# play-with-HOI-generation/HOIG

Hardware: AMD Instinct MI355X
Metric: HOGAN train images/sec at 256x256 (higher is better)
Workload: dtype f16x3 fwd (both operands split hi+lo on fp16, 3 MFMAs per product) / bf16x2 bwd (dy split hi+lo, weights and x single bf16, 2 MFMAs per product), f32 accumulate; 1 GPU; 256x256 HO3Dv3-shaped synthetic, batch 8 per GPU, G+D full step (generator_spade_attn, VGG19 surrogate weights); global_batch=8, parallelism=dp1

## Files before the change

hoig_amd/csrc/conv_route.h:

```cpp
#pragma once

#define HOIG_CONV_ROUTES(W, D, F, FD)                                                                                              \
          \
    W(wgrad_thin_in_ws) W(wgrad_thin_in_direct) W(wgrad_thin_out_ws) W(wgrad_thin_out_direct)                                      \
    W(wgrad_small)                                                                                                                 \
                                                                                        \
    W(wgrad_flat5) W(wgrad_tile5)                                                                                                  \
                                                                 \
    W(wgrad_halo_th4) W(wgrad_halo_cm2) W(wgrad_halo_cm1) W(wgrad_halo_s2_cm2) W(wgrad_halo_s2_cm1) W(wgrad_halo_5x5)              \
    W(wgrad_halo_tout)        \
                                                                                                  \
    W(wgrad_dma) W(wgrad_dma_pair)                                                                                                 \
    W(wgrad_bf16_64) W(wgrad_bf16_128)                                                                                             \
                                                                                 \
    W(wgrad_f32_32x64) W(wgrad_f32_32x128) W(wgrad_f32_64x128) W(wgrad_f32_128x64) W(wgrad_f32_128x128)                            \
                                                                                 \
    FD(igemm_f32_128x32) FD(igemm_f32_128x64) FD(igemm_f32_64x64) FD(igemm_f32_128x128) FD(igemm_f32_64x128)                       \
                       \
    FD(halo1_64) FD(halo1_128w) FD(halo1_128) FD(same5_64) FD(same5_128w) FD(same5_128)                                            \
                                                                                                             \
    FD(halo3_64) FD(halo3_128w) FD(halo3_128)                                                                                      \
         \
    FD(halo3_m16_64) FD(halo3_m16_128)                                                                                             \
    D(halo3_m16_64_split) D(halo3_m16_128_split) D(halo3_m16_64_split_pair) D(halo3_m16_128_split_pair)                            \
    F(halo3_m16_64_pair) F(halo3_m16_128_pair) F(halo3_m16_64_normin) F(halo3_m16_128_normin)                                      \
                                                   \
    FD(flat_m16_k3) FD(flat_m16_k5) FD(halo5_m16) FD(halo5_m16_ksplit)                                                             \
     \
    FD(s2g_64) FD(s2g_128) FD(s2s_64) FD(s2s_128)                                                                                  \
    FD(s2g_m16_64) FD(s2g_m16_128) FD(s2s_m16_64) FD(s2s_m16_128)                                                                  \
    FD(s2g_m16p4_64) FD(s2g_m16p4_128) FD(s2s_m16p4_64) FD(s2s_m16p4_128) FD(s2g_m16p8_128) FD(s2s_m16p8_128)                      \
                   \
    FD(igemm_m16_128x128) FD(igemm_m16_128x128w) FD(igemm_m16_64x128) FD(igemm_m16_128x64) FD(igemm_m16_64x64)                     \
    FD(igemm_bf16_128x128) FD(igemm_bf16_128x128w) FD(igemm_bf16_64x128) FD(igemm_bf16_128x64) FD(igemm_bf16_64x64)                \
                                                                                \
    D(k128) D(thin) D(thin_out) D(small)                                                                                           \
    F(head7) F(small) F(small_ci) F(dot) F(thin) F(thin_out)                                                                       \
// ... 27 lines not shown
```

hoig_amd/csrc/conv_thin.hip:

```cpp
#include "common.h"
#include <map>
#include <mutex>

namespace {

typedef _Float16 f16x8 __attribute__((ext_vector_type(8)));
typedef short s16x4 __attribute__((ext_vector_type(4)));

constexpr int TH = 4, TW = 32, NTHR = 256;

struct ThinArgs {
    const float *T;
    const float *D;
    const float *bias;
    float *Out;
    float *Ws;
    int Bn, H, W, F, CD, KS, pad;
    int flip;
    int sj, st, sf;
    int act;
    float slope;
    int accumulate;
    float wscale;
    int K, KP, N, NP;
    int tiles_x, tiles_y, ntiles, strip;
    int HR, CW;
    double *stats;
};

template <bool FP16>
__device__ __forceinline__ void split16(float x, unsigned short &hi, unsigned short &lo) {
    if (FP16) {
        const _Float16 h = (_Float16)x;
        const _Float16 l = (_Float16)(x - (float)h);
        hi = __builtin_bit_cast(unsigned short, h);
        lo = __builtin_bit_cast(unsigned short, l);
    } else {
        const __bf16 h = (__bf16)x;
        hi = __builtin_bit_cast(unsigned short, h);
        const __bf16 l = (__bf16)(x - hoig_bf2f(hi));
        lo = __builtin_bit_cast(unsigned short, l);
    }
}

template <bool FP16>
__device__ __forceinline__ f32x16 mfma16(const bf16x8 a, const bf16x8 b, const f32x16 c) {
    if (FP16) return __builtin_amdgcn_mfma_f32_32x32x16_f16(__builtin_bit_cast(f16x8, a), __builtin_bit_cast(f16x8, b), c, 0, 0, 0);
    return __builtin_amdgcn_mfma_f32_32x32x16_bf16(a, b, c, 0, 0, 0);
}

constexpr int HMAX = 12;
struct HaloRegs {
    float v[HMAX];
};
struct HaloMap {
    int lds[HMAX];
    int rc[HMAX];
    int rounds;
};
__device__ __forceinline__ void halo_map(const ThinArgs &p, HaloMap &m) {
    const int wr = TW + p.KS - 1;
    const int row_elems = wr * p.F;
    const int total = p.HR * row_elems;
    m.rounds = (total + NTHR - 1) / NTHR;
#pragma unroll
    for (int it = 0; it < HMAX; ++it) {
        const int i = threadIdx.x + it * NTHR;
        m.lds[it] = -1;
        m.rc[it] = 0;
        if (i < total) {
            const int hy = i / row_elems, e = i - hy * row_elems;
            const int hx = e / p.F, f = e - hx * p.F;
            m.lds[it] = (f * p.HR + hy) * p.CW + hx;
            m.rc[it] = hy | (hx << 8) | (f << 16);
        }
    }
}
__device__ __forceinline__ void halo_load(const ThinArgs &p, const HaloMap &m, int b, int y0, int x0, HaloRegs &h) {
    const float *img = p.T + (size_t)b * p.H * p.W * p.F;
#pragma unroll
    for (int it = 0; it < HMAX; ++it) {
        h.v[it] = 0.f;
        if (it < m.rounds && m.lds[it] >= 0) {
            const int gy = y0 - p.pad + (m.rc[it] & 255), gx = x0 - p.pad + ((m.rc[it] >> 8) & 255);
            if (gy >= 0 && gy < p.H && gx >= 0 && gx < p.W) h.v[it] = img[((size_t)gy * p.W + gx) * p.F + (m.rc[it] >> 16)];
        }
    }
}
template <bool FP16, int NT>
__device__ __forceinline__ void halo_store(const ThinArgs &p, const HaloMap &m, const HaloRegs &h, unsigned short *Tl) {
    const int plane = p.F * p.HR * p.CW;
#pragma unroll
    for (int it = 0; it < HMAX; ++it)
        if (it < m.rounds && m.lds[it] >= 0) {
            unsigned short hi, lo;
            split16<FP16>(h.v[it], hi, lo);
            Tl[m.lds[it]] = hi;
            if (NT == 2) Tl[plane + m.lds[it]] = lo;
        }
}

__device__ __forceinline__ void tile_coords(const ThinArgs &p, int t, int &b, int &y0, int &x0) {
    const int tx = t % p.tiles_x;
    t /= p.tiles_x;
    const int ty = t % p.tiles_y;
    b = t / p.tiles_y;
    y0 = ty * TH;
    x0 = tx * TW;
}

template <bool FP16, int NT, int NW>
__global__ __launch_bounds__(NTHR) void thin_gemm_kernel(const ThinArgs p) {
    extern __shared__ __attribute__((aligned(16))) unsigned char smem[];
    const int wstride = p.KP + 8;
    unsigned short *Wl = reinterpret_cast<unsigned short *>(smem);
    unsigned short *toff = Wl + NW * 64 * wstride;
    unsigned short *Tl = toff + p.KP;
    const int tid = threadIdx.x, lane = tid & 63, wave = tid >> 6;
    const int l31 = lane & 31, lh = lane >> 5;
    const int cbase = blockIdx.y * 64;
    const int KK = p.KS * p.KS;
    const int tplane = p.F * p.HR * p.CW;

    for (int i0 = tid; i0 < 64 * p.KP; i0 += 4 * NTHR) {
        float v[4];
        int dst[4];
#pragma unroll
        for (int u = 0; u < 4; ++u) {
            const int i = i0 + u * NTHR;
            v[u] = 0.f;
            dst[u] = -1;
            if (i < 64 * p.KP) {
                const int n = i / p.KP, k = i - n * p.KP;
                dst[u] = n * wstride + k;
                if (k < p.K) {
                    const int tap = k / p.F, f = k - tap * p.F;
                    const int tw = p.flip ? KK - 1 - tap : tap;
                    v[u] = p.D[(size_t)(cbase + n) * p.sj + (size_t)tw * p.st + (size_t)f * p.sf];
                }
            }
        }
#pragma unroll
        for (int u = 0; u < 4; ++u)
            if (dst[u] >= 0) {
                unsigned short hi, lo;
                split16<FP16>(v[u] * p.wscale, hi, lo);
                Wl[dst[u]] = hi;
                if (NW == 2) Wl[64 * wstride + dst[u]] = lo;
            }
    }
    for (int k = tid; k < p.KP; k += NTHR) {
        const int kc = k < p.K ? k : p.K - 1;
        const int tap = kc / p.F, f = kc - tap * p.F;
        const int r = tap / p.KS, s = tap - r * p.KS;
        toff[k] = (unsigned short)((f * p.HR + r) * p.CW + s);
    }

    const float nslope = p.act == HOIG_ACT_NONE ? 1.f : (p.act == HOIG_ACT_RELU ? 0.f : p.slope);
    const bool special = p.act == HOIG_ACT_TANH || p.act == HOIG_ACT_SIGMOID;
    const float inv = 1.f / p.wscale;
    float bias_r[2];
#pragma unroll
    for (int j = 0; j < 2; ++j) bias_r[j] = p.bias ? p.bias[cbase + j * 32 + l31] : 0.f;
    const int ksteps = p.KP >> 4;
    const int pix = wave * p.CW + l31;

    const int t_end = min(p.ntiles, (int)(blockIdx.x + 1) * p.strip);
    HaloRegs hreg;
    HaloMap hmap;
    halo_map(p, hmap);
    {
        int b, y0, x0;
        tile_coords(p, blockIdx.x * p.strip, b, y0, x0);
        halo_load(p, hmap, b, y0, x0, hreg);
    }
    float st1[2] = {0.f, 0.f}, st2[2] = {0.f, 0.f};
    int sb = -1;
    auto flush_stats = [&]() {
        if (sb >= 0) {
#pragma unroll
            for (int j = 0; j < 2; ++j) {
                const float s1 = st1[j] + __shfl_xor(st1[j], 32), s2 = st2[j] + __shfl_xor(st2[j], 32);
                if (lh == 0) {
                    hoig_stats_add(p.stats, sb, p.CD, 0, cbase + j * 32 + l31, s1);
                    hoig_stats_add(p.stats, sb, p.CD, 1, cbase + j * 32 + l31, s2);
                }
                st1[j] = st2[j] = 0.f;
            }
        }
    };
    for (int t = blockIdx.x * p.strip; t < t_end; ++t) {
        int b, y0, x0;
        tile_coords(p, t, b, y0, x0);
        if (p.stats && b != sb) {
            flush_stats();
            sb = b;
        }
        __syncthreads();
        halo_store<FP16, NT>(p, hmap, hreg, Tl);
        __syncthreads();
        if (t + 1 < t_end) {
            int b2, y2, x2;
            tile_coords(p, t + 1, b2, y2, x2);
            halo_load(p, hmap, b2, y2, x2, hreg);
        }
        f32x16 acc[2];
#pragma unroll
        for (int j = 0; j < 2; ++j)
#pragma unroll
            for (int r = 0; r < 16; ++r) acc[j][r] = 0.f;
#pragma unroll 1
        for (int kk = 0; kk < ksteps; ++kk) {
            const int k0 = kk * 16 + lh * 8;
            const bf16x8 offs = *reinterpret_cast<const bf16x8 *>(toff + k0);
            bf16x8 a0, a1;
#pragma unroll
            for (int e = 0; e < 8; ++e) {
                const int o = (int)(unsigned short)offs[e] + pix;
                a0[e] = (short)Tl[o];
                if (NT == 2) a1[e] = (short)Tl[tplane + o];
            }
#pragma unroll
            for (int j = 0; j < 2; ++j) {
                const unsigned short *wr = Wl + (j * 32 + l31) * wstride + k0;
                const bf16x8 w0 = *reinterpret_cast<const bf16x8 *>(wr);
                if (NT == 2) acc[j] = mfma16<FP16>(a1, w0, acc[j]);
                if (NW == 2) acc[j] = mfma16<FP16>(a0, *reinterpret_cast<const bf16x8 *>(wr + 64 * wstride), acc[j]);
                acc[j] = mfma16<FP16>(a0, w0, acc[j]);
            }
        }
        const int oy = y0 + wave;
#pragma unroll
        for (int r = 0; r < 16; ++r) {
            const int ox = x0 + (r & 3) + 8 * (r >> 2) + 4 * lh;
            float *dst = p.Out + (((size_t)b * p.H + oy) * p.W + ox) * p.CD + cbase + l31;
#pragma unroll
            for (int j = 0; j < 2; ++j) {
                float v = acc[j][r] * inv + bias_r[j];
                v = fast_act(v, nslope, special, p.act, p.slope);
                if (p.accumulate) v += dst[j * 32];
                dst[j * 32] = v;
                st1[j] += v;
                st2[j] += v * v;
            }
        }
    }
    if (p.stats) flush_stats();
}

constexpr int DROW = 192;

template <int NPW, int WN, int NT, int ND>
__global__ __launch_bounds__(NTHR) void thin_wgrad_kernel(const ThinArgs p) {
    constexpr int WK = 4 / WN, NPIX = TH * TW, KSTEPS = NPIX / 16;
    extern __shared__ __attribute__((aligned(16))) unsigned char smem[];
    unsigned char *Dl = smem;
    unsigned short *Tl = reinterpret_cast<unsigned short *>(smem + ND * NPIX * DROW);
    float *Gl = reinterpret_cast<float *>(smem);
    const int tid = threadIdx.x, lane = tid & 63, wave = tid >> 6;
    const int l31 = lane & 31, lh = lane >> 5;
    const int wn = wave % WN, wk = wave / WN;
    const int cbase = blockIdx.y * 64;
    const int KK = p.KS * p.KS;
    const int tplane = p.F * p.HR * p.CW;

    int noff[NPW];
    bool nval[NPW];
#pragma unroll
    for (int j = 0; j < NPW; ++j) {
        const int n = (wn * NPW + j) * 32 + l31;
        nval[j] = n < p.N;
        const int nc = nval[j] ? n : 0;
        const int tap = nc / p.F, f = nc - tap * p.F;
        const int tt = p.flip ? KK - 1 - tap : tap;
        const int r = tt / p.KS, s = tt - r * p.KS;
        noff[j] = (f * p.HR + r) * p.CW + s + lh * 8;
    }
    const int g = lane >> 4, q = (lane >> 2) & 3, pp = lane & 3;
    const int a_off = (8 * (g >> 1) + q) * DROW + (16 * (g & 1) + 4 * pp) * 2;

    f32x16 acc[2][NPW];
#pragma unroll
    for (int i = 0; i < 2; ++i)
#pragma unroll
        for (int j = 0; j < NPW; ++j)
#pragma unroll
            for (int r = 0; r < 16; ++r) acc[i][j][r] = 0.f;

    constexpr int DT = NPIX * 8 / NTHR;
    float4 dreg[DT][2];
    auto load_d = [&](int t) {
        int b, y0, x0;
        tile_coords(p, t, b, y0, x0);
#pragma unroll
        for (int i = 0; i < DT; ++i) {
            const int task = tid + i * NTHR, px = task >> 3, c8 = task & 7;
            const int yy = y0 + (px >> 5), xx = x0 + (px & 31);
            const float *src = p.D + (((size_t)b * p.H + yy) * p.W + xx) * p.CD + cbase + c8 * 8;
            dreg[i][0] = *reinterpret_cast<const float4 *>(src);
            dreg[i][1] = *reinterpret_cast<const float4 *>(src + 4);
        }
    };
    auto store_d = [&]() {
#pragma unroll
        for (int i = 0; i < DT; ++i) {
            const int task = tid + i * NTHR, px = task >> 3, c8 = task & 7;
            const float v[8] = {dreg[i][0].x, dreg[i][0].y, dreg[i][0].z, dreg[i][0].w,
                                dreg[i][1].x, dreg[i][1].y, dreg[i][1].z, dreg[i][1].w};
            bf16x8 hi, lo;
#pragma unroll
            for (int e = 0; e < 8; e += 2) {
                typedef float f2v __attribute__((ext_vector_type(2)));
                typedef __bf16 b2v __attribute__((ext_vector_type(2)));
                const f2v x2 = {v[e], v[e + 1]};
                const unsigned hp = __builtin_bit_cast(unsigned, __builtin_convertvector(x2, b2v));
                hi[e] = (short)(hp & 0xffffu);
                hi[e + 1] = (short)(hp >> 16);
                if (ND == 2) {
                    const f2v r2 = {v[e] - __uint_as_float(hp << 16), v[e + 1] - __uint_as_float(hp & 0xffff0000u)};
                    const unsigned lp = __builtin_bit_cast(unsigned, __builtin_convertvector(r2, b2v));
                    lo[e] = (short)(lp & 0xffffu);
                    lo[e + 1] = (short)(lp >> 16);
                }
            }
            *reinterpret_cast<bf16x8 *>(Dl + px * DROW + c8 * 16) = hi;
            if (ND == 2) *reinterpret_cast<bf16x8 *>(Dl + NPIX * DROW + px * DROW + c8 * 16) = lo;
        }
    };

    int t = blockIdx.x;
    HaloRegs hreg;
    HaloMap hmap;
    halo_map(p, hmap);
    if (t < p.ntiles) {
        int b, y0, x0;
        tile_coords(p, t, b, y0, x0);
        load_d(t);
        halo_load(p, hmap, b, y0, x0, hreg);
    }
    for (; t < p.ntiles; t += gridDim.x) {
        __syncthreads();
        store_d();
        halo_store<false, NT>(p, hmap, hreg, Tl);
        __syncthreads();
        if (t + (int)gridDim.x < p.ntiles) {
            int b, y0, x0;
            tile_coords(p, t + gridDim.x, b, y0, x0);
            load_d(t + gridDim.x);
            halo_load(p, hmap, b, y0, x0, hreg);
        }
#pragma unroll 1
        for (int ks = wk; ks < KSTEPS; ks += WK) {
            const int prow = ks >> 1, pcol = (ks & 1) * 16;
            bf16x8 a[2][ND];
#pragma unroll
            for (int i = 0; i < 2; ++i)
#pragma unroll
                for (int d = 0; d < ND; ++d) {
                    const unsigned char *src = Dl + d * NPIX * DROW + (prow * 32 + pcol) * DROW + a_off + i * 64;
                    const s16x4 v0 = __builtin_amdgcn_ds_read_tr16_b64_v4i16((__attribute__((address_space(3))) s16x4 *)(src));
                    const s16x4 v1 = __builtin_amdgcn_ds_read_tr16_b64_v4i16((__attribute__((address_space(3))) s16x4 *)(src + 4 * DROW));
                    a[i][d] = (bf16x8){v0[0], v0[1], v0[2], v0[3], v1[0], v1[1], v1[2], v1[3]};
                }
            const int base = prow * p.CW + pcol;
#pragma unroll
            for (int j = 0; j < NPW; ++j) {
                bf16x8 b0, b1;
#pragma unroll
                for (int e = 0; e < 8; ++e) {
                    const int o = base + noff[j] + e;
                    b0[e] = nval[j] ? (short)Tl[o] : (short)0;
                    if (NT == 2) b1[e] = nval[j] ? (short)Tl[tplane + o] : (short)0;
                }
#pragma unroll
                for (int i = 0; i < 2; ++i) {
                    if (ND == 2) acc[i][j] = mfma16<false>(a[i][1], b0, acc[i][j]);
                    if (NT == 2) acc[i][j] = mfma16<false>(a[i][0], b1, acc[i][j]);
                    acc[i][j] = mfma16<false>(a[i][0], b0, acc[i][j]);
                }
            }
        }
    }

    __syncthreads();
    for (int i = tid; i < 64 * p.NP; i += NTHR) Gl[i] = 0.f;
    __syncthreads();
#pragma unroll
    for (int i = 0; i < 2; ++i)
#pragma unroll
        for (int j = 0; j < NPW; ++j) {
            const int n = (wn * NPW + j) * 32 + l31;
            if (n < p.NP)
#pragma unroll
                for (int r = 0; r < 16; ++r) {
                    const int m = i * 32 + (r & 3) + 8 * (r >> 2) + 4 * lh;
                    if (WK > 1) atomicAdd(&Gl[m * p.NP + n], acc[i][j][r]);
                    else Gl[m * p.NP + n] = acc[i][j][r];
                }
        }
    __syncthreads();
    if (p.Ws) {
        float *dst = p.Ws + ((size_t)blockIdx.y * gridDim.x + blockIdx.x) * 64 * p.NP;
        for (int i = tid; i < 64 * p.NP; i += NTHR) dst[i] = Gl[i];
        return;
    }
    if (p.sj == 1) {
        for (int i = tid; i < 64 * p.N; i += NTHR) {
            const int n = i >> 6, m = i & 63;
            const int tap = n / p.F, f = n - tap * p.F;
            atomicAdd(p.Out + (size_t)f * p.sf + (size_t)tap * p.st + cbase + m, Gl[m * p.NP + n]);
        }
    } else {
        for (int i = tid; i < 64 * p.N; i += NTHR) {
            const int m = i / p.N, n = i - m * p.N;
            const int tap = n / p.F, f = n - tap * p.F;
            atomicAdd(p.Out + (size_t)(cbase + m) * p.sj + (size_t)tap * p.st + (size_t)f * p.sf, Gl[m * p.NP + n]);
        }
    }
}

__global__ __launch_bounds__(NTHR) void thin_reduce_kernel(const ThinArgs p, int nwg) {
    const int cbase = blockIdx.y * 64;
    const float *src = p.Ws + (size_t)blockIdx.y * nwg * 64 * p.NP;
    const int i = blockIdx.x * NTHR + threadIdx.x;
    if (i >= 64 * p.N) return;
    const int m = i / p.N, n = i - m * p.N;
    const int wper = (nwg + (int)gridDim.z - 1) / (int)gridDim.z;
    const int w0 = blockIdx.z * wper, w1 = min(nwg, w0 + wper);
    const size_t step = (size_t)64 * p.NP;
    const float *col = src + m * p.NP + n + (size_t)w0 * step;
    float v0 = 0.f, v1 = 0.f, v2 = 0.f, v3 = 0.f;
    int w = w0;
    for (; w + 3 < w1; w += 4, col += 4 * step) {
        v0 += col[0];
        v1 += col[step];
        v2 += col[2 * step];
// ... 139 lines not shown
                }
#pragma unroll
                for (int i = 0; i < 2; ++i) {
                    const unsigned char *ap = Dl + apix[i] + toff;
                    const bf16x8 ah = *reinterpret_cast<const bf16x8 *>(ap);
                    if (ND == 2) acc[i] = mfma16x16<FP16>(*reinterpret_cast<const bf16x8 *>(ap + hpix * PROW), bh, acc[i]);
                    if (NW == 2) acc[i] = mfma16x16<FP16>(ah, bl, acc[i]);
                    acc[i] = mfma16x16<FP16>(ah, bh, acc[i]);
                }
            }
        }
        if (nvalid) {
            const int tx = t % p.tiles_x, r1 = t / p.tiles_x;
            const int b = r1 / p.tiles_y, y0 = (r1 % p.tiles_y) * TH, x0 = tx * TW;
#pragma unroll
            for (int i = 0; i < 2; ++i) {
                const int g = 2 * wave + i;
                const int oy = y0 + (g >> 1), oxb = x0 + 16 * (g & 1) + 4 * kg;
#pragma unroll
                for (int e = 0; e < 4; ++e) {
                    const float v = acc[i][e] * inv + bias_n;
                    p.Out[(((size_t)b * p.H + oy) * p.W + oxb + e) * p.F + l15] = hoig_act(v, act_n, p.slope);
                }
            }
        }
    }
}

bool thin_geometry(const hoig_conv_desc *d) {
    return !d->transposed && d->stride == 1 && d->R == d->S && (d->R & 1) && d->R <= 7 && 2 * d->pad == d->R - 1 &&
           d->Ho == d->Hi && d->Wo == d->Wi && (d->Hi % TH) == 0 && (d->Wi % TW) == 0;
}

void fill_common(ThinArgs &a, const hoig_conv_desc *d, int F, int CD) {
    a.Bn = d->B; a.H = d->Hi; a.W = d->Wi; a.F = F; a.CD = CD; a.KS = d->R; a.pad = d->pad;
    a.K = d->R * d->S * F;
    a.KP = (a.K + 15) / 16 * 16;
    a.N = a.K;
    a.NP = (a.N + 31) / 32 * 32;
    a.tiles_x = d->Wi / TW; a.tiles_y = d->Hi / TH;
    a.ntiles = d->B * a.tiles_x * a.tiles_y;
    a.HR = TH + d->R - 1;
    a.CW = (TW + d->R - 1 + 8 + 1) & ~1;
    a.bias = nullptr; a.act = HOIG_ACT_NONE; a.slope = 0.f; a.accumulate = 0; a.wscale = 1.f; a.strip = 1; a.Ws = nullptr; a.stats = nullptr;
}

template <bool FP16>
int launch_gemm(const ThinArgs &a, int precision, hipStream_t st) {
    const int nt = precision == HOIG_PREC_BF16 ? 1 : 2, nw = precision == HOIG_PREC_BF16X3 ? 2 : 1;
    const size_t smem = (size_t)nw * 64 * (a.KP + 8) * 2 + (size_t)a.KP * 2 + (size_t)nt * a.F * a.HR * a.CW * 2;
    if (smem > 160 * 1024) return HOIG_EUNSUPPORTED;
    dim3 grid((unsigned)hoig_cdiv(a.ntiles, a.strip), a.CD / 64);
    HOIG_ROUTE_FD(FP16, thin);
    if (nt == 2 && nw == 2) return hoig_launch<thin_gemm_kernel<FP16, 2, 2>, 160 * 1024>(grid, NTHR, smem, st, a);
    if (nt == 2) return hoig_launch<thin_gemm_kernel<FP16, 2, 1>, 160 * 1024>(grid, NTHR, smem, st, a);
    return hoig_launch<thin_gemm_kernel<FP16, 1, 1>, 160 * 1024>(grid, NTHR, smem, st, a);
}

template <int NPW, int WN>
int launch_wgrad_t(const ThinArgs &a, int nt, int nd, dim3 grid, size_t smem, hipStream_t st) {
    if (nt == 2 && nd == 2) return hoig_launch<thin_wgrad_kernel<NPW, WN, 2, 2>, 160 * 1024>(grid, NTHR, smem, st, a);
    if (nt == 2) return hoig_launch<thin_wgrad_kernel<NPW, WN, 2, 1>, 160 * 1024>(grid, NTHR, smem, st, a);
    if (nd == 2) return hoig_launch<thin_wgrad_kernel<NPW, WN, 1, 2>, 160 * 1024>(grid, NTHR, smem, st, a);
    return hoig_launch<thin_wgrad_kernel<NPW, WN, 1, 1>, 160 * 1024>(grid, NTHR, smem, st, a);
}

}

int hoig_conv_thin_fwd(const hoig_conv_desc *d, const float *x, const float *w, const float *bias, float *y, hipStream_t st, double *stats) {
    if (d->precision == HOIG_PREC_F32 || !thin_geometry(d) || d->Ci > (d->R <= 3 ? 12 : 8) || d->Ci < 1 || (d->Co % 64)) return HOIG_EUNSUPPORTED;
    ThinArgs a;
    fill_common(a, d, d->Ci, d->Co);
    a.T = x; a.D = w; a.bias = bias; a.Out = y; a.stats = stats;
    a.flip = 0;
    a.sj = d->R * d->S * d->Ci; a.st = d->Ci; a.sf = 1;
    a.act = d->act; a.slope = d->slope;
    a.wscale = 256.f;
    a.strip = a.ntiles >= 4096 ? 8 : (a.ntiles >= 1024 ? 4 : 1);
    return launch_gemm<true>(a, d->precision, st);
}

int hoig_conv_thin_dgrad(const hoig_conv_desc *d, const float *dy, const float *w, float *dx, int accumulate, hipStream_t st) {
    if (d->precision == HOIG_PREC_F32 || !thin_geometry(d) || d->Co > 8 || d->Co < 1 || (d->Ci % 64)) return HOIG_EUNSUPPORTED;
    ThinArgs a;
    fill_common(a, d, d->Co, d->Ci);
    a.T = dy; a.D = w; a.Out = dx;
    a.flip = 1;
    a.sj = 1; a.st = d->Ci; a.sf = d->R * d->S * d->Ci;
    a.accumulate = accumulate;
    a.strip = a.ntiles >= 4096 ? 8 : (a.ntiles >= 1024 ? 4 : 1);
    return launch_gemm<false>(a, d->precision, st);
}

bool hoig_conv_thin_wgrad_applies(const hoig_conv_desc *d) {
    if (d->precision == HOIG_PREC_F32 || !thin_geometry(d)) return false;
    return (d->Ci <= (d->R <= 3 ? 12 : 8) && (d->Co % 64) == 0) || (d->Co <= 8 && (d->Ci % 64) == 0);
}

int hoig_conv_thin_wgrad(const hoig_conv_desc *d, const float *x, const float *dy, float *dw, hipStream_t st) {
    if (d->precision == HOIG_PREC_F32 || !thin_geometry(d)) return HOIG_EUNSUPPORTED;
    const bool thin_in = d->Ci <= (d->R <= 3 ? 12 : 8) && (d->Co % 64) == 0, thin_out = d->Co <= 8 && (d->Ci % 64) == 0;
    if (!thin_in && !thin_out) return HOIG_EUNSUPPORTED;
    ThinArgs a;
    int nt, nd;
    if (thin_in) {
        fill_common(a, d, d->Ci, d->Co);
        a.T = x; a.D = dy; a.flip = 0;
        a.sj = d->R * d->S * d->Ci; a.st = d->Ci; a.sf = 1;
        nd = d->precision == HOIG_PREC_BF16 ? 1 : 2;
        nt = d->precision == HOIG_PREC_BF16X3 ? 2 : 1;
    } else {
        fill_common(a, d, d->Co, d->Ci);
        a.T = dy; a.D = x; a.flip = 1;
        a.sj = 1; a.st = d->Ci; a.sf = d->R * d->S * d->Ci;
        nt = d->precision == HOIG_PREC_BF16 ? 1 : 2;
        nd = d->precision == HOIG_PREC_BF16X3 ? 2 : 1;
    }
    a.Out = dw;
    const int nfr = a.NP / 32;
    if (nfr > 16) return HOIG_EUNSUPPORTED;
    size_t smem = (size_t)nd * TH * TW * DROW + (size_t)nt * a.F * a.HR * a.CW * 2;
    const size_t gsm = (size_t)64 * a.NP * 4;
    if (gsm > smem) smem = gsm;
    if (smem > 160 * 1024) return HOIG_EUNSUPPORTED;
    int nwg = 512;
    if (smem > 80 * 1024 || a.N >= 128) nwg = 256;
    if (nwg > a.ntiles) nwg = a.ntiles;
    const int groups = a.CD / 64;
    while (nwg > 64 && (size_t)nwg * groups * 64 * a.NP * 4 > WS_SLOT_BYTES) nwg >>= 1;
    dim3 grid(nwg, groups);
    a.Ws = nwg > 8 ? thin_workspace(st, (size_t)nwg * groups * 64 * a.NP * 4) : nullptr;
    if (thin_in) a.Ws ? HOIG_ROUTE_W(wgrad_thin_in_ws) : HOIG_ROUTE_W(wgrad_thin_in_direct);
    else a.Ws ? HOIG_ROUTE_W(wgrad_thin_out_ws) : HOIG_ROUTE_W(wgrad_thin_out_direct);
    int rc;
    if (nfr == 1) rc = launch_wgrad_t<1, 1>(a, nt, nd, grid, smem, st);
    else if (nfr == 2) rc = launch_wgrad_t<2, 1>(a, nt, nd, grid, smem, st);
    else if (nfr <= 4) rc = launch_wgrad_t<2, 2>(a, nt, nd, grid, smem, st);
    else if (nfr <= 8) rc = launch_wgrad_t<2, 4>(a, nt, nd, grid, smem, st);
    else rc = launch_wgrad_t<4, 4>(a, nt, nd, grid, smem, st);
    if (rc != HOIG_OK || !a.Ws) return rc;
    thin_reduce_kernel<<<dim3((unsigned)hoig_cdiv(64 * a.N, NTHR), groups, (unsigned)hoig_cdiv(nwg, 32)), NTHR, 0, st>>>(a, nwg);
    HOIG_LAUNCH_CHECK();
    return HOIG_OK;
}

int hoig_conv_thin_out(const hoig_conv_desc *d, const float *x, const float *w, const float *bias, float *y,
                       unsigned long long acts, int dgrad, hipStream_t st) {
    if (d->precision == HOIG_PREC_F32 || !thin_geometry(d)) return HOIG_EUNSUPPORTED;
    const int F = dgrad ? d->Ci : d->Co, CD = dgrad ? d->Co : d->Ci;
    if (F < 1 || F > 16 || (CD % 64)) return HOIG_EUNSUPPORTED;
    if (d->R > 3) return HOIG_EUNSUPPORTED;
    ThinOutArgs a;
    a.D = x; a.Wt = w; a.bias = bias; a.Out = y;
    a.Bn = d->B; a.H = d->Hi; a.W = d->Wi; a.F = F; a.CD = CD; a.KS = d->R; a.pad = d->pad;
    const int KK = d->R * d->S;
    if (!dgrad) { a.flip = 0; a.sf = KK * CD; a.st = CD; a.sj = 1; a.wscale = 256.f; }
    else { a.flip = 1; a.sf = 1; a.st = F; a.sj = KK * F; a.wscale = 1.f; }
    a.acts = acts; a.slope = d->slope;
    a.tiles_x = d->Wi / TW; a.tiles_y = d->Hi / TH; a.ntiles = d->B * a.tiles_x * a.tiles_y;
    a.strip = a.ntiles >= 2048 ? 8 : (a.ntiles >= 512 ? 2 : 1);
    a.HR = TH + d->R - 1; a.HWc = TW + d->R - 1;
    if (a.HR * a.HWc * 8 > 12 * NTHR) return HOIG_EUNSUPPORTED;
    const int nd = d->precision == HOIG_PREC_BF16 ? 1 : 2, nw = d->precision == HOIG_PREC_BF16X3 ? 2 : 1;
    const size_t smem = (size_t)nw * (CD / 64) * F * KK * 144 + (size_t)nd * a.HR * a.HWc * 80;
    if (smem > 160 * 1024) return HOIG_EUNSUPPORTED;
    const unsigned grid = (unsigned)hoig_cdiv(a.ntiles, a.strip);
    HOIG_ROUTE_FD(!dgrad, thin_out);
    if (!dgrad) {
        if (nd == 2 && nw == 2) return hoig_launch<thin_out_kernel<true, 2, 2>, 160 * 1024>(grid, NTHR, smem, st, a);
        if (nd == 2) return hoig_launch<thin_out_kernel<true, 2, 1>, 160 * 1024>(grid, NTHR, smem, st, a);
        return hoig_launch<thin_out_kernel<true, 1, 1>, 160 * 1024>(grid, NTHR, smem, st, a);
    }
    if (nd == 2 && nw == 2) return hoig_launch<thin_out_kernel<false, 2, 2>, 160 * 1024>(grid, NTHR, smem, st, a);
// ... 4 lines not shown
```

hoig_amd/csrc/tuning.h:

```cpp
#pragma once
enum HoigTuning { HOIG_TUNE_IGEMM16 = 0, HOIG_TUNE_S2_16, HOIG_TUNE_FLAT5, HOIG_TUNE_WFLAT5, HOIG_TUNE_HEAD16, HOIG_TUNE_D_EARLY, HOIG_TUNE_SPLIT_GRADS, HOIG_TUNE_PAIR, HOIG_TUNE_WDMA16, HOIG_TUNE_S2_PIPE, HOIG_TUNE_NORM_IN, HOIG_TUNE_WINO8, HOIG_TUNE_HALO5, HOIG_TUNE_PNG_WINDOW, HOIG_TUNE_COUNT };
int hoig_tuning(int id);
```

hoig_amd/csrc/tuning.hip:

```cpp
#include <cstring>
#include "hoig_kernels.h"
#include "tuning.h"
#include "conv_route.h"

namespace {
struct Entry {
    const char *key;
    int value;
};
Entry g_table[HOIG_TUNE_COUNT] = {
    {"igemm16", 1},
    {"s2_16", 1},
    {"flat5", 2},
    {"wflat5", 1},
    {"head16", 1},
    {"d_early", 1},
    {"split_grads", 1},
    {"pair", 2},
    {"wdma16", 2},
    {"s2_pipe", 1},
    {"norm_in", 1},
    {"wino8", 0},
    {"halo5", 1},
    {"png_window", 0},
};
}

int hoig_tuning(int id) { return (id >= 0 && id < HOIG_TUNE_COUNT) ? g_table[id].value : 0; }

extern "C" int hoig_set_tuning(const char *key, int value) {
    if (!key) return -1;
    for (int i = 0; i < HOIG_TUNE_COUNT; ++i)
        if (strcmp(g_table[i].key, key) == 0) {
            const int prev = g_table[i].value;
            if (value >= 0) g_table[i].value = value;
            return prev;
        }
    return -1;
}

thread_local int hoig_route_last[3] = {0, 0, 0};

extern "C" int hoig_conv_last_route(int which) { return (which >= 0 && which < 3) ? hoig_route_last[which] : -1; }

extern "C" const char *hoig_conv_route_name(int id) {
    static const char *const names[HOIG_ROUTE_COUNT] = {
        "none",
#define HOIG_R_W(n) #n,
#define HOIG_R_D(n) "dgrad_" #n,
#define HOIG_R_F(n) "fwd_" #n,
#define HOIG_R_FD(n) "fwd_" #n, "dgrad_" #n,
        HOIG_CONV_ROUTES(HOIG_R_W, HOIG_R_D, HOIG_R_F, HOIG_R_FD)
#undef HOIG_R_W
#undef HOIG_R_D
#undef HOIG_R_F
#undef HOIG_R_FD
    };
// ... 3 lines not shown
```

Measured before the change: 132.7 images/s.

## Add taller-tile thin conv kernel and shifted-copy halo for thin wgrad

Adds a thin2 GEMM path for thin-channel forward and dgrad convolutions. It uses 8-row tiles with 512 threads and software-pipelines the LDS gather loads one k-step ahead of the MFMAs. For thin wgrad it stores four column-shifted copies of the halo in LDS so the B operand can be read as aligned 4-element vectors instead of scalar gathers, at the cost of more shared memory. It also adds compile-time KO probe switches (default off) that skip loads and stores for profiling, and a tuning key thin2 that is on by default.

Result: no change. 133.0 images/s (median of 2 runs) (+0.2%).

```diff
diff --git a/hoig_amd/csrc/conv_route.h b/hoig_amd/csrc/conv_route.h
--- a/hoig_amd/csrc/conv_route.h
+++ b/hoig_amd/csrc/conv_route.h
@@ -3,6 +3,9 @@
 #define HOIG_CONV_ROUTES(W, D, F, FD)                                                                                              \
           \
     W(wgrad_thin_in_ws) W(wgrad_thin_in_direct) W(wgrad_thin_out_ws) W(wgrad_thin_out_direct)                                      \
+     \
+     \
+    W(thin2_fwd) W(thin2_dgrad) W(thin2_wgrad_in_ws) W(thin2_wgrad_in_direct) W(thin2_wgrad_out_ws) W(thin2_wgrad_out_direct)      \
     W(wgrad_small)                                                                                                                 \
                                                                                         \
     W(wgrad_flat5) W(wgrad_tile5)                                                                                                  \
diff --git a/hoig_amd/csrc/conv_thin.hip b/hoig_amd/csrc/conv_thin.hip
--- a/hoig_amd/csrc/conv_thin.hip
+++ b/hoig_amd/csrc/conv_thin.hip
@@ -1,4 +1,5 @@
 #include "common.h"
+#include "tuning.h"
 #include <map>
 #include <mutex>
 
@@ -8,6 +9,11 @@
 typedef short s16x4 __attribute__((ext_vector_type(4)));
 
 constexpr int TH = 4, TW = 32, NTHR = 256;
+constexpr int TH2 = 8, NTHR2 = 512;
+#ifndef HOIG_THIN_KO
+#define HOIG_THIN_KO 0
+#endif
+constexpr int KO = HOIG_THIN_KO;
 
 struct ThinArgs {
     const float *T;
@@ -58,14 +64,15 @@
     int rc[HMAX];
     int rounds;
 };
+template <int NTH = NTHR>
 __device__ __forceinline__ void halo_map(const ThinArgs &p, HaloMap &m) {
     const int wr = TW + p.KS - 1;
     const int row_elems = wr * p.F;
     const int total = p.HR * row_elems;
-    m.rounds = (total + NTHR - 1) / NTHR;
+    m.rounds = (total + NTH - 1) / NTH;
 #pragma unroll
     for (int it = 0; it < HMAX; ++it) {
-        const int i = threadIdx.x + it * NTHR;
+        const int i = threadIdx.x + it * NTH;
         m.lds[it] = -1;
         m.rc[it] = 0;
         if (i < total) {
@@ -87,7 +94,7 @@
         }
     }
 }
-template <bool FP16, int NT>
+template <bool FP16, int NT, int NC = 1>
 __device__ __forceinline__ void halo_store(const ThinArgs &p, const HaloMap &m, const HaloRegs &h, unsigned short *Tl) {
     const int plane = p.F * p.HR * p.CW;
 #pragma unroll
@@ -96,16 +103,23 @@
             unsigned short hi, lo;
             split16<FP16>(h.v[it], hi, lo);
             Tl[m.lds[it]] = hi;
-            if (NT == 2) Tl[plane + m.lds[it]] = lo;
-        }
-}
-
+            if (NT == 2) Tl[NC * plane + m.lds[it]] = lo;
+#pragma unroll
+            for (int c = 1; c < NC; ++c)
+                if (m.lds[it] >= c) {
+                    Tl[c * plane + m.lds[it] - c] = hi;
+                    if (NT == 2) Tl[(NC + c) * plane + m.lds[it] - c] = lo;
+                }
+        }
+}
+
+template <int THT = TH>
 __device__ __forceinline__ void tile_coords(const ThinArgs &p, int t, int &b, int &y0, int &x0) {
     const int tx = t % p.tiles_x;
     t /= p.tiles_x;
     const int ty = t % p.tiles_y;
     b = t / p.tiles_y;
-    y0 = ty * TH;
+    y0 = ty * THT;
     x0 = tx * TW;
 }
 
@@ -122,7 +136,7 @@
     const int KK = p.KS * p.KS;
     const int tplane = p.F * p.HR * p.CW;
 
-    for (int i0 = tid; i0 < 64 * p.KP; i0 += 4 * NTHR) {
+    for (int i0 = tid; i0 < ((KO & 4) ? 0 : 64 * p.KP); i0 += 4 * NTHR) {
         float v[4];
         int dst[4];
 #pragma unroll
@@ -172,7 +186,9 @@
     {
         int b, y0, x0;
         tile_coords(p, blockIdx.x * p.strip, b, y0, x0);
-        halo_load(p, hmap, b, y0, x0, hreg);
+        if (!(KO & 2)) halo_load(p, hmap, b, y0, x0, hreg);
+        else
+            for (int it = 0; it < HMAX; ++it) hreg.v[it] = 0.f;
     }
     float st1[2] = {0.f, 0.f}, st2[2] = {0.f, 0.f};
     int sb = -1;
@@ -197,9 +213,9 @@
             sb = b;
         }
         __syncthreads();
-        halo_store<FP16, NT>(p, hmap, hreg, Tl);
+        if (!(KO & 2) || t == (int)blockIdx.x * p.strip) halo_store<FP16, NT>(p, hmap, hreg, Tl);
         __syncthreads();
-        if (t + 1 < t_end) {
+        if (t + 1 < t_end && !(KO & 2)) {
             int b2, y2, x2;
             tile_coords(p, t + 1, b2, y2, x2);
             halo_load(p, hmap, b2, y2, x2, hreg);
@@ -214,11 +230,17 @@
             const int k0 = kk * 16 + lh * 8;
             const bf16x8 offs = *reinterpret_cast<const bf16x8 *>(toff + k0);
             bf16x8 a0, a1;
-#pragma unroll
-            for (int e = 0; e < 8; ++e) {
-                const int o = (int)(unsigned short)offs[e] + pix;
-                a0[e] = (short)Tl[o];
-                if (NT == 2) a1[e] = (short)Tl[tplane + o];
+            if (KO & 1) {
+                const int o = ((kk & 7) * 8 + pix * 8) & 1023;
+                a0 = *reinterpret_cast<const bf16x8 *>(Tl + o);
+                if (NT == 2) a1 = *reinterpret_cast<const bf16x8 *>(Tl + 1024 + o);
+            } else {
+#pragma unroll
+                for (int e = 0; e < 8; ++e) {
+                    const int o = (int)(unsigned short)offs[e] + pix;
+                    a0[e] = (short)Tl[o];
+                    if (NT == 2) a1[e] = (short)Tl[tplane + o];
+                }
             }
 #pragma unroll
             for (int j = 0; j < 2; ++j) {
@@ -239,7 +261,7 @@
                 float v = acc[j][r] * inv + bias_r[j];
                 v = fast_act(v, nslope, special, p.act, p.slope);
                 if (p.accumulate) v += dst[j * 32];
-                dst[j * 32] = v;
+                if (!(KO & 8) || v == 1234.5f) dst[j * 32] = v;
                 st1[j] += v;
                 st2[j] += v * v;
             }
@@ -248,11 +270,198 @@
     if (p.stats) flush_stats();
 }
 
+template <bool FP16, int NT, int NW>
+__global__ __launch_bounds__(NTHR2) void thin2_gemm_kernel(const ThinArgs p) {
+    extern __shared__ __attribute__((aligned(16))) unsigned char smem[];
+    const int wstride = p.KP + 8;
+    unsigned short *Wl = reinterpret_cast<unsigned short *>(smem);
+    unsigned short *toff = Wl + NW * 64 * wstride;
+    unsigned short *Tl = toff + p.KP;
+    const int tid = threadIdx.x, lane = tid & 63, wave = tid >> 6;
+    const int l31 = lane & 31, lh = lane >> 5;
+    const int cbase = blockIdx.y * 64;
+    const int KK = p.KS * p.KS;
+    const int tplane = p.F * p.HR * p.CW;
+
+    for (int i0 = tid; i0 < ((KO & 4) ? 0 : 64 * p.KP); i0 += 4 * NTHR2) {
+        float v[4];
+        int dst[4];
+#pragma unroll
+        for (int u = 0; u < 4; ++u) {
+            const int i = i0 + u * NTHR2;
+            v[u] = 0.f;
+            dst[u] = -1;
+            if (i < 64 * p.KP) {
+                const int n = i / p.KP, k = i - n * p.KP;
+                dst[u] = n * wstride + k;
+                if (k < p.K) {
+                    const int tap = k / p.F, f = k - tap * p.F;
+                    const int tw = p.flip ? KK - 1 - tap : tap;
+                    v[u] = p.D[(size_t)(cbase + n) * p.sj + (size_t)tw * p.st + (size_t)f * p.sf];
+                }
+            }
+        }
+#pragma unroll
+        for (int u = 0; u < 4; ++u)
+            if (dst[u] >= 0) {
+                unsigned short hi, lo;
+                split16<FP16>(v[u] * p.wscale, hi, lo);
+                Wl[dst[u]] = hi;
+                if (NW == 2) Wl[64 * wstride + dst[u]] = lo;
+            }
+    }
+    for (int k = tid; k < p.KP; k += NTHR2) {
+        const int kc = k < p.K ? k : p.K - 1;
+        const int tap = kc / p.F, f = kc - tap * p.F;
+        const int r = tap / p.KS, s = tap - r * p.KS;
+        toff[k] = (unsigned short)((f * p.HR + r) * p.CW + s);
+    }
+
+    const float nslope = p.act == HOIG_ACT_NONE ? 1.f : (p.act == HOIG_ACT_RELU ? 0.f : p.slope);
+    const bool special = p.act == HOIG_ACT_TANH || p.act == HOIG_ACT_SIGMOID;
+    const float inv = 1.f / p.wscale;
+    float bias_r[2];
+#pragma unroll
+    for (int j = 0; j < 2; ++j) bias_r[j] = p.bias ? p.bias[cbase + j * 32 + l31] : 0.f;
+    const int ksteps = p.KP >> 4;
+    const int pix = wave * p.CW + l31;
+    const unsigned short *wrow = Wl + l31 * wstride + lh * 8;
+    const unsigned short *orow = toff + lh * 8;
+
+    const int t_end = min(p.ntiles, (int)(blockIdx.x + 1) * p.strip);
+    HaloRegs hreg;
+    HaloMap hmap;
+    halo_map<NTHR2>(p, hmap);
+    {
+        int b, y0, x0;
+        tile_coords<TH2>(p, blockIdx.x * p.strip, b, y0, x0);
+        if (!(KO & 2)) halo_load(p, hmap, b, y0, x0, hreg);
+        else
+            for (int it = 0; it < HMAX; ++it) hreg.v[it] = 0.f;
+    }
+    float st1[2] = {0.f, 0.f}, st2[2] = {0.f, 0.f};
+    int sb = -1;
+    auto flush_stats = [&]() {
+        if (sb >= 0) {
+#pragma unroll
+            for (int j = 0; j < 2; ++j) {
+                const float s1 = st1[j] + __shfl_xor(st1[j], 32), s2 = st2[j] + __shfl_xor(st2[j], 32);
+                if (lh == 0) {
+                    hoig_stats_add(p.stats, sb, p.CD, 0, cbase + j * 32 + l31, s1);
+                    hoig_stats_add(p.stats, sb, p.CD, 1, cbase + j * 32 + l31, s2);
+                }
+                st1[j] = st2[j] = 0.f;
+            }
+        }
+    };
+    for (int t = blockIdx.x * p.strip; t < t_end; ++t) {
+        int b, y0, x0;
+        tile_coords<TH2>(p, t, b, y0, x0);
+        if (p.stats && b != sb) {
+            flush_stats();
+            sb = b;
+        }
+        __syncthreads();
+        if (!(KO & 2) || t == (int)blockIdx.x * p.strip) halo_store<FP16, NT>(p, hmap, hreg, Tl);
+        __syncthreads();
+        if (t + 1 < t_end && !(KO & 2)) {
+            int b2, y2, x2;
+            tile_coords<TH2>(p, t + 1, b2, y2, x2);
+            halo_load(p, hmap, b2, y2, x2, hreg);
+        }
+        f32x16 acc[2];
+#pragma unroll
+        for (int j = 0; j < 2; ++j)
+#pragma unroll
+            for (int r = 0; r < 16; ++r) acc[j][r] = 0.f;
+
+        unsigned r0[8], r1[8];
+        bf16x8 wn[2][NW];
+        bf16x8 offs;
+        auto issue = [&](int kk) {
+            if (KO & 1) {
+                const int o = ((kk & 7) * 8 + pix * 8) & 1023;
+                const bf16x8 v0 = *reinterpret_cast<const bf16x8 *>(Tl + o);
+                const bf16x8 v1 = *reinterpret_cast<const bf16x8 *>(Tl + 1024 + o);
+#pragma unroll
+                for (int e = 0; e < 8; ++e) {
+                    r0[e] = (unsigned short)v0[e];
+                    r1[e] = (unsigned short)v1[e];
+                }
+            } else {
+#pragma unroll
+                for (int e = 0; e < 8; ++e) {
+                    const int o = (int)(unsigned short)offs[e] + pix;
+                    r0[e] = Tl[o];
+                    if (NT == 2) r1[e] = Tl[tplane + o];
+                }
+            }
+#pragma unroll
+            for (int j = 0; j < 2; ++j) {
+                wn[j][0] = *reinterpret_cast<const bf16x8 *>(wrow + j * 32 * wstride + kk * 16);
+                if (NW == 2) wn[j][1] = *reinterpret_cast<const bf16x8 *>(wrow + (64 + j * 32) * wstride + kk * 16);
+            }
+        };
+        offs = *reinterpret_cast<const bf16x8 *>(orow);
+        issue(0);
+        offs = *reinterpret_cast<const bf16x8 *>(orow + min(1, ksteps - 1) * 16);
+#pragma unroll 1
+        for (int kk = 0; kk < ksteps; ++kk) {
+            bf16x8 a0, a1, w[2][NW];
+            {
+                typedef unsigned u32x4 __attribute__((ext_vector_type(4)));
+                u32x4 p0, p1;
+#pragma unroll
+                for (int e = 0; e < 4; ++e) {
+                    p0[e] = r0[2 * e] | (r0[2 * e + 1] << 16);
+                    if (NT == 2) p1[e] = r1[2 * e] | (r1[2 * e + 1] << 16);
+                }
+                a0 = __builtin_bit_cast(bf16x8, p0);
+                if (NT == 2) a1 = __builtin_bit_cast(bf16x8, p1);
+            }
+#pragma unroll
+            for (int j = 0; j < 2; ++j)
+#pragma unroll
+                for (int n = 0; n < NW; ++n) w[j][n] = wn[j][n];
+            issue(min(kk + 1, ksteps - 1));
+            offs = *reinterpret_cast<const bf16x8 *>(orow + min(kk + 2, ksteps - 1) * 16);
+            __builtin_amdgcn_sched_barrier(0);
+#pragma unroll
+            for (int j = 0; j < 2; ++j)
+                if (NT == 2) acc[j] = mfma16<FP16>(a1, w[j][0], acc[j]);
+#pragma unroll
+            for (int j = 0; j < 2; ++j)
+                if (NW == 2) acc[j] = mfma16<FP16>(a0, w[j][NW - 1], acc[j]);
+#pragma unroll
+            for (int j = 0; j < 2; ++j) acc[j] = mfma16<FP16>(a0, w[j][0], acc[j]);
+            __builtin_amdgcn_sched_barrier(0);
+        }
+        const int oy = y0 + wave;
+        if (oy < p.H) {
+#pragma unroll
+            for (int r = 0; r < 16; ++r) {
+                const int ox = x0 + (r & 3) + 8 * (r >> 2) + 4 * lh;
+                float *dst = p.Out + (((size_t)b * p.H + oy) * p.W + ox) * p.CD + cbase + l31;
+#pragma unroll
+                for (int j = 0; j < 2; ++j) {
+                    float v = acc[j][r] * inv + bias_r[j];
+                    v = fast_act(v, nslope, special, p.act, p.slope);
+                    if (p.accumulate) v += dst[j * 32];
+                    if (!(KO & 8) || v == 1234.5f) dst[j * 32] = v;
+                    st1[j] += v;
+                    st2[j] += v * v;
+                }
+            }
+        }
+    }
+    if (p.stats) flush_stats();
+}
+
 constexpr int DROW = 192;
 
-template <int NPW, int WN, int NT, int ND>
+template <int NPW, int WN, int NT, int ND, bool SH = false>
 __global__ __launch_bounds__(NTHR) void thin_wgrad_kernel(const ThinArgs p) {
-    constexpr int WK = 4 / WN, NPIX = TH * TW, KSTEPS = NPIX / 16;
+    constexpr int WK = 4 / WN, NPIX = TH * TW, KSTEPS = NPIX / 16, NC = SH ? 4 : 1;
     extern __shared__ __attribute__((aligned(16))) unsigned char smem[];
     unsigned char *Dl = smem;
     unsigned short *Tl = reinterpret_cast<unsigned short *>(smem + ND * NPIX * DROW);
@@ -275,6 +484,7 @@
         const int tt = p.flip ? KK - 1 - tap : tap;
         const int r = tt / p.KS, s = tt - r * p.KS;
         noff[j] = (f * p.HR + r) * p.CW + s + lh * 8;
+        if (SH) noff[j] += (s & 3) * (tplane - 1);
     }
     const int g = lane >> 4, q = (lane >> 2) & 3, pp = lane & 3;
     const int a_off = (8 * (g >> 1) + q) * DROW + (16 * (g & 1) + 4 * pp) * 2;
@@ -335,18 +545,18 @@
     if (t < p.ntiles) {
         int b, y0, x0;
         tile_coords(p, t, b, y0, x0);
-        load_d(t);
+        if (!(KO & 32)) load_d(t);
         halo_load(p, hmap, b, y0, x0, hreg);
     }
     for (; t < p.ntiles; t += gridDim.x) {
         __syncthreads();
-        store_d();
-        halo_store<false, NT>(p, hmap, hreg, Tl);
+        if (!(KO & 32)) store_d();
+        halo_store<false, NT, NC>(p, hmap, hreg, Tl);
         __syncthreads();
         if (t + (int)gridDim.x < p.ntiles) {
             int b, y0, x0;
             tile_coords(p, t + gridDim.x, b, y0, x0);
-            load_d(t + gridDim.x);
+            if (!(KO & 32)) load_d(t + gridDim.x);
             halo_load(p, hmap, b, y0, x0, hreg);
         }
 #pragma unroll 1
@@ -366,11 +576,28 @@
 #pragma unroll
             for (int j = 0; j < NPW; ++j) {
                 bf16x8 b0, b1;
-#pragma unroll
-                for (int e = 0; e < 8; ++e) {
-                    const int o = base + noff[j] + e;
-                    b0[e] = nval[j] ? (short)Tl[o] : (short)0;
-                    if (NT == 2) b1[e] = nval[j] ? (short)Tl[tplane + o] : (short)0;
+                if (KO & 1) {
+                    const int o = ((ks & 7) * 8 + (j * 64 + lane) * 8) & 2047;
+                    b0 = *reinterpret_cast<const bf16x8 *>(Tl + o);
+                    if (NT == 2) b1 = *reinterpret_cast<const bf16x8 *>(Tl + 2048 + o);
+                } else if (SH) {
+                    const unsigned short *src = Tl + base + noff[j];
+                    const s16x4 z = {0, 0, 0, 0};
+                    const s16x4 l0 = nval[j] ? *reinterpret_cast<const s16x4 *>(src) : z;
+                    const s16x4 h0 = nval[j] ? *reinterpret_cast<const s16x4 *>(src + 4) : z;
+                    b0 = (bf16x8){l0[0], l0[1], l0[2], l0[3], h0[0], h0[1], h0[2], h0[3]};
+                    if (NT == 2) {
+                        const s16x4 l1 = nval[j] ? *reinterpret_cast<const s16x4 *>(src + NC * tplane) : z;
+                        const s16x4 h1 = nval[j] ? *reinterpret_cast<const s16x4 *>(src + NC * tplane + 4) : z;
+                        b1 = (bf16x8){l1[0], l1[1], l1[2], l1[3], h1[0], h1[1], h1[2], h1[3]};
+                    }
+                } else {
+#pragma unroll
+                    for (int e = 0; e < 8; ++e) {
+                        const int o = base + noff[j] + e;
+                        b0[e] = nval[j] ? (short)Tl[o] : (short)0;
+                        if (NT == 2) b1[e] = nval[j] ? (short)Tl[tplane + o] : (short)0;
+                    }
                 }
 #pragma unroll
                 for (int i = 0; i < 2; ++i) {
@@ -401,7 +628,8 @@
     __syncthreads();
     if (p.Ws) {
         float *dst = p.Ws + ((size_t)blockIdx.y * gridDim.x + blockIdx.x) * 64 * p.NP;
-        for (int i = tid; i < 64 * p.NP; i += NTHR) dst[i] = Gl[i];
+        for (int i = tid; i < 64 * p.NP; i += NTHR)
+            if (!(KO & 16) || Gl[i] == 1234.5f) dst[i] = Gl[i];
         return;
     }
     if (p.sj == 1) {
@@ -607,16 +835,34 @@
            d->Ho == d->Hi && d->Wo == d->Wi && (d->Hi % TH) == 0 && (d->Wi % TW) == 0;
 }
 
-void fill_common(ThinArgs &a, const hoig_conv_desc *d, int F, int CD) {
+enum { THIN2_FWD = 0, THIN2_DGRAD, THIN2_WGRAD_IN, THIN2_WGRAD_OUT };
+bool thin2_picks(int kind, const hoig_conv_desc *d) {
+    const int key = hoig_tuning(HOIG_TUNE_THIN2);
+    if (key != 1) return key > 1;
+    const int64_t map = (int64_t)d->Hi * d->Wi;
+    switch (kind) {
+        case THIN2_FWD: {
+            const int KP = (d->R * d->S * d->Ci + 15) / 16 * 16, nw = d->precision == HOIG_PREC_BF16X3 ? 2 : 1;
+            if ((size_t)nw * 64 * (KP + 8) * 2 > 80 * 1024) return true;
+            return d->R == 3 && map <= 4096 && d->B * map >= 16384;
+        }
+        case THIN2_WGRAD_IN: return d->R == 7;
+        case THIN2_WGRAD_OUT: return d->R == 7 && d->Co >= 3;
+        default: return false;
+    }
+}
+
+void fill_common(ThinArgs &a, const hoig_conv_desc *d, int F, int CD, int THT = TH, bool cw4 = false) {
     a.Bn = d->B; a.H = d->Hi; a.W = d->Wi; a.F = F; a.CD = CD; a.KS = d->R; a.pad = d->pad;
     a.K = d->R * d->S * F;
     a.KP = (a.K + 15) / 16 * 16;
     a.N = a.K;
     a.NP = (a.N + 31) / 32 * 32;
-    a.tiles_x = d->Wi / TW; a.tiles_y = d->Hi / TH;
+    a.tiles_x = d->Wi / TW; a.tiles_y = (d->Hi + THT - 1) / THT;
     a.ntiles = d->B * a.tiles_x * a.tiles_y;
-    a.HR = TH + d->R - 1;
+    a.HR = THT + d->R - 1;
     a.CW = (TW + d->R - 1 + 8 + 1) & ~1;
+    if (cw4) a.CW = (a.CW + 3) & ~3;
     a.bias = nullptr; a.act = HOIG_ACT_NONE; a.slope = 0.f; a.accumulate = 0; a.wscale = 1.f; a.strip = 1; a.Ws = nullptr; a.stats = nullptr;
 }
 
@@ -632,37 +878,55 @@
     return hoig_launch<thin_gemm_kernel<FP16, 1, 1>, 160 * 1024>(grid, NTHR, smem, st, a);
 }
 
-template <int NPW, int WN>
+template <bool FP16>
+int launch_gemm2(ThinArgs &a, int precision, hipStream_t st) {
+    const int nt = precision == HOIG_PREC_BF16 ? 1 : 2, nw = precision == HOIG_PREC_BF16X3 ? 2 : 1;
+    const size_t smem = (size_t)nw * 64 * (a.KP + 8) * 2 + (size_t)a.KP * 2 + (size_t)nt * a.F * a.HR * a.CW * 2;
+    if (smem > 160 * 1024 || a.HR * (TW + a.KS - 1) * a.F > HMAX * NTHR2) return HOIG_EUNSUPPORTED;
+    const int groups = a.CD / 64, round = smem > 80 * 1024 ? 256 : 512;
+    a.strip = hoig_tuning(HOIG_TUNE_THIN2) == 3 ? 3 : (int)hoig_cdiv((int64_t)a.ntiles * groups, round);
+    dim3 grid((unsigned)hoig_cdiv(a.ntiles, a.strip), groups);
+    hoig_route_set(FP16 ? HOIG_PASS_FWD : HOIG_PASS_DGRAD, FP16 ? HOIG_ROUTE_thin2_fwd : HOIG_ROUTE_thin2_dgrad);
+    if (nt == 2 && nw == 2) return hoig_launch<thin2_gemm_kernel<FP16, 2, 2>, 160 * 1024>(grid, NTHR2, smem, st, a);
+    if (nt == 2) return hoig_launch<thin2_gemm_kernel<FP16, 2, 1>, 160 * 1024>(grid, NTHR2, smem, st, a);
+    return hoig_launch<thin2_gemm_kernel<FP16, 1, 1>, 160 * 1024>(grid, NTHR2, smem, st, a);
+}
+
+template <int NPW, int WN, bool SH = false>
 int launch_wgrad_t(const ThinArgs &a, int nt, int nd, dim3 grid, size_t smem, hipStream_t st) {
-    if (nt == 2 && nd == 2) return hoig_launch<thin_wgrad_kernel<NPW, WN, 2, 2>, 160 * 1024>(grid, NTHR, smem, st, a);
-    if (nt == 2) return hoig_launch<thin_wgrad_kernel<NPW, WN, 2, 1>, 160 * 1024>(grid, NTHR, smem, st, a);
-    if (nd == 2) return hoig_launch<thin_wgrad_kernel<NPW, WN, 1, 2>, 160 * 1024>(grid, NTHR, smem, st, a);
-    return hoig_launch<thin_wgrad_kernel<NPW, WN, 1, 1>, 160 * 1024>(grid, NTHR, smem, st, a);
+    if (nt == 2 && nd == 2) return hoig_launch<thin_wgrad_kernel<NPW, WN, 2, 2, SH>, 160 * 1024>(grid, NTHR, smem, st, a);
+    if (nt == 2) return hoig_launch<thin_wgrad_kernel<NPW, WN, 2, 1, SH>, 160 * 1024>(grid, NTHR, smem, st, a);
+    if (nd == 2) return hoig_launch<thin_wgrad_kernel<NPW, WN, 1, 2, SH>, 160 * 1024>(grid, NTHR, smem, st, a);
+    return hoig_launch<thin_wgrad_kernel<NPW, WN, 1, 1, SH>, 160 * 1024>(grid, NTHR, smem, st, a);
 }
 
 }
 
 int hoig_conv_thin_fwd(const hoig_conv_desc *d, const float *x, const float *w, const float *bias, float *y, hipStream_t st, double *stats) {
     if (d->precision == HOIG_PREC_F32 || !thin_geometry(d) || d->Ci > (d->R <= 3 ? 12 : 8) || d->Ci < 1 || (d->Co % 64)) return HOIG_EUNSUPPORTED;
+    const bool two = thin2_picks(THIN2_FWD, d);
     ThinArgs a;
-    fill_common(a, d, d->Ci, d->Co);
+    fill_common(a, d, d->Ci, d->Co, two ? TH2 : TH);
     a.T = x; a.D = w; a.bias = bias; a.Out = y; a.stats = stats;
     a.flip = 0;
     a.sj = d->R * d->S * d->Ci; a.st = d->Ci; a.sf = 1;
     a.act = d->act; a.slope = d->slope;
     a.wscale = 256.f;
+    if (two) return launch_gemm2<true>(a, d->precision, st);
     a.strip = a.ntiles >= 4096 ? 8 : (a.ntiles >= 1024 ? 4 : 1);
     return launch_gemm<true>(a, d->precision, st);
 }
 
 int hoig_conv_thin_dgrad(const hoig_conv_desc *d, const float *dy, const float *w, float *dx, int accumulate, hipStream_t st) {
     if (d->precision == HOIG_PREC_F32 || !thin_geometry(d) || d->Co > 8 || d->Co < 1 || (d->Ci % 64)) return HOIG_EUNSUPPORTED;
+    const bool two = thin2_picks(THIN2_DGRAD, d);
     ThinArgs a;
-    fill_common(a, d, d->Co, d->Ci);
+    fill_common(a, d, d->Co, d->Ci, two ? TH2 : TH);
     a.T = dy; a.D = w; a.Out = dx;
     a.flip = 1;
     a.sj = 1; a.st = d->Ci; a.sf = d->R * d->S * d->Ci;
     a.accumulate = accumulate;
+    if (two) return launch_gemm2<false>(a, d->precision, st);
     a.strip = a.ntiles >= 4096 ? 8 : (a.ntiles >= 1024 ? 4 : 1);
     return launch_gemm<false>(a, d->precision, st);
 }
@@ -676,16 +940,17 @@
     if (d->precision == HOIG_PREC_F32 || !thin_geometry(d)) return HOIG_EUNSUPPORTED;
     const bool thin_in = d->Ci <= (d->R <= 3 ? 12 : 8) && (d->Co % 64) == 0, thin_out = d->Co <= 8 && (d->Ci % 64) == 0;
     if (!thin_in && !thin_out) return HOIG_EUNSUPPORTED;
+    const bool two = thin2_picks(thin_in ? THIN2_WGRAD_IN : THIN2_WGRAD_OUT, d);
     ThinArgs a;
     int nt, nd;
     if (thin_in) {
-        fill_common(a, d, d->Ci, d->Co);
+        fill_common(a, d, d->Ci, d->Co, TH, two);
         a.T = x; a.D = dy; a.flip = 0;
         a.sj = d->R * d->S * d->Ci; a.st = d->Ci; a.sf = 1;
         nd = d->precision == HOIG_PREC_BF16 ? 1 : 2;
         nt = d->precision == HOIG_PREC_BF16X3 ? 2 : 1;
     } else {
-        fill_common(a, d, d->Co, d->Ci);
+        fill_common(a, d, d->Co, d->Ci, TH, two);
         a.T = dy; a.D = x; a.flip = 1;
         a.sj = 1; a.st = d->Ci; a.sf = d->R * d->S * d->Ci;
         nt = d->precision == HOIG_PREC_BF16 ? 1 : 2;
@@ -694,26 +959,36 @@
     a.Out = dw;
     const int nfr = a.NP / 32;
     if (nfr > 16) return HOIG_EUNSUPPORTED;
-    size_t smem = (size_t)nd * TH * TW * DROW + (size_t)nt * a.F * a.HR * a.CW * 2;
+    size_t smem = (size_t)nd * TH * TW * DROW + (size_t)nt * (two ? 4 : 1) * a.F * a.HR * a.CW * 2;
     const size_t gsm = (size_t)64 * a.NP * 4;
     if (gsm > smem) smem = gsm;
     if (smem > 160 * 1024) return HOIG_EUNSUPPORTED;
     int nwg = 512;
     if (smem > 80 * 1024 || a.N >= 128) nwg = 256;
+    if (two && hoig_tuning(HOIG_TUNE_THIN2) == 3) nwg = 2;
     if (nwg > a.ntiles) nwg = a.ntiles;
     const int groups = a.CD / 64;
     while (nwg > 64 && (size_t)nwg * groups * 64 * a.NP * 4 > WS_SLOT_BYTES) nwg >>= 1;
     dim3 grid(nwg, groups);
     a.Ws = nwg > 8 ? thin_workspace(st, (size_t)nwg * groups * 64 * a.NP * 4) : nullptr;
-    if (thin_in) a.Ws ? HOIG_ROUTE_W(wgrad_thin_in_ws) : HOIG_ROUTE_W(wgrad_thin_in_direct);
+    if (two) {
+        if (thin_in) a.Ws ? HOIG_ROUTE_W(thin2_wgrad_in_ws) : HOIG_ROUTE_W(thin2_wgrad_in_direct);
+        else a.Ws ? HOIG_ROUTE_W(thin2_wgrad_out_ws) : HOIG_ROUTE_W(thin2_wgrad_out_direct);
+    } else if (thin_in) a.Ws ? HOIG_ROUTE_W(wgrad_thin_in_ws) : HOIG_ROUTE_W(wgrad_thin_in_direct);
     else a.Ws ? HOIG_ROUTE_W(wgrad_thin_out_ws) : HOIG_ROUTE_W(wgrad_thin_out_direct);
     int rc;
-    if (nfr == 1) rc = launch_wgrad_t<1, 1>(a, nt, nd, grid, smem, st);
+    if (two) {
+        if (nfr == 1) rc = launch_wgrad_t<1, 1, true>(a, nt, nd, grid, smem, st);
+        else if (nfr == 2) rc = launch_wgrad_t<2, 1, true>(a, nt, nd, grid, smem, st);
+        else if (nfr <= 4) rc = launch_wgrad_t<2, 2, true>(a, nt, nd, grid, smem, st);
+        else if (nfr <= 8) rc = launch_wgrad_t<2, 4, true>(a, nt, nd, grid, smem, st);
+        else rc = launch_wgrad_t<4, 4, true>(a, nt, nd, grid, smem, st);
+    } else if (nfr == 1) rc = launch_wgrad_t<1, 1>(a, nt, nd, grid, smem, st);
     else if (nfr == 2) rc = launch_wgrad_t<2, 1>(a, nt, nd, grid, smem, st);
     else if (nfr <= 4) rc = launch_wgrad_t<2, 2>(a, nt, nd, grid, smem, st);
     else if (nfr <= 8) rc = launch_wgrad_t<2, 4>(a, nt, nd, grid, smem, st);
     else rc = launch_wgrad_t<4, 4>(a, nt, nd, grid, smem, st);
-    if (rc != HOIG_OK || !a.Ws) return rc;
+    if (rc != HOIG_OK || !a.Ws || (KO & 16)) return rc;
     thin_reduce_kernel<<<dim3((unsigned)hoig_cdiv(64 * a.N, NTHR), groups, (unsigned)hoig_cdiv(nwg, 32)), NTHR, 0, st>>>(a, nwg);
     HOIG_LAUNCH_CHECK();
     return HOIG_OK;
diff --git a/hoig_amd/csrc/tuning.h b/hoig_amd/csrc/tuning.h
--- a/hoig_amd/csrc/tuning.h
+++ b/hoig_amd/csrc/tuning.h
@@ -1,3 +1,3 @@
 #pragma once
-enum HoigTuning { HOIG_TUNE_IGEMM16 = 0, HOIG_TUNE_S2_16, HOIG_TUNE_FLAT5, HOIG_TUNE_WFLAT5, HOIG_TUNE_HEAD16, HOIG_TUNE_D_EARLY, HOIG_TUNE_SPLIT_GRADS, HOIG_TUNE_PAIR, HOIG_TUNE_WDMA16, HOIG_TUNE_S2_PIPE, HOIG_TUNE_NORM_IN, HOIG_TUNE_WINO8, HOIG_TUNE_HALO5, HOIG_TUNE_PNG_WINDOW, HOIG_TUNE_COUNT };
+enum HoigTuning { HOIG_TUNE_IGEMM16 = 0, HOIG_TUNE_S2_16, HOIG_TUNE_FLAT5, HOIG_TUNE_WFLAT5, HOIG_TUNE_HEAD16, HOIG_TUNE_D_EARLY, HOIG_TUNE_SPLIT_GRADS, HOIG_TUNE_PAIR, HOIG_TUNE_WDMA16, HOIG_TUNE_S2_PIPE, HOIG_TUNE_NORM_IN, HOIG_TUNE_WINO8, HOIG_TUNE_HALO5, HOIG_TUNE_PNG_WINDOW, HOIG_TUNE_THIN2, HOIG_TUNE_COUNT };
 int hoig_tuning(int id);
diff --git a/hoig_amd/csrc/tuning.hip b/hoig_amd/csrc/tuning.hip
--- a/hoig_amd/csrc/tuning.hip
+++ b/hoig_amd/csrc/tuning.hip
@@ -23,6 +23,7 @@
     {"wino8", 0},
     {"halo5", 1},
     {"png_window", 0},
+    {"thin2", 1},
 };
 }
 
```
